# ParthaEth/GIF

Hardware: NVIDIA H100
Metric: G+D train step images/sec @256x256 bs32/GPU (higher is better)
Workload: dtype bf16x3 error-compensated tensor-core contraction (two-term bf16 operands, 3 MMAs per slice), f32 accumulate/storage

## Files before the change

### gif_b200/_lib.py

```python
import ctypes
import os

import torch

_HERE = os.path.dirname(os.path.abspath(__file__))
LIB_PATH = os.path.join(_HERE, "libgifb200.so")

_p = ctypes.c_void_p
_i = ctypes.c_int
_f = ctypes.c_float
_d = ctypes.c_double
_ll = ctypes.c_longlong
_sz = ctypes.c_size_t

SIGNATURES = {
    "gifb200_version": (_i, []),
    "gifb200_last_error": (ctypes.c_char_p, []),
    "gifb200_launch_count": (_ll, []),
    "gifb200_conv2d_workspace_bytes": (_sz, [_i] * 11),
    "gifb200_conv2d": (_i, [_p, _p, _p] + [_i] * 13 + [_p, _f, _f, _i, _p, _sz, _p]),
    "gifb200_conv2d_wgrad_workspace_bytes": (_sz, [_i] * 10),
    "gifb200_conv2d_wgrad_path": (_i, [_i] * 10),
    "gifb200_conv2d_wgrad": (_i, [_p, _p, _p] + [_i] * 12 + [_p, _sz, _p]),
    "gifb200_conv2d_ex_workspace_bytes": (_sz, [_i] * 13),
    "gifb200_conv2d_ex": (_i, [_p, _p, _p] + [_i] * 16 + [_p, _i, _p, _sz, _p]),
    "gifb200_pool2d": (_i, [_p, _p] + [_i] * 12 + [_p]),
    "gifb200_resize_bilinear": (_i, [_p, _p, _i, _i, _i, _ll, _ll, _ll, _ll, _i, _i, _i, _f, _f, _i, _p]),
    "gifb200_resize_bilinear_u8": (_i, [_p, _p, _i, _i, _i, _ll, _i, _i, _i, _f, _f, _i, _p]),
    "gifb200_split_bf16": (_i, [_p, _p, _p, _i, _i, _i, _p]),
    "gifb200_upfirdn2d": (_i, [_p, _p, _p] + [_i] * 14 + [_p]),
    "gifb200_bias_act": (_i, [_p, _p, _p, _p, _p, _i, _i, _i, _f, _f, _i, _p]),
    "gifb200_act_bwd": (_i, [_p, _p, _p, _ll, _f, _f, _i, _p]),
    "gifb200_rows_sum": (_i, [_p, _p, _i, _i, _i, _p]),
    "gifb200_chan_scale": (_i, [_p, _p, _p, _i, _i, _i, _i, _p]),
    "gifb200_tail_bwd": (_i, [_p] * 8 + [_i, _i, _i, _f, _f, _i, _p]),
    "gifb200_tail_bwd_planes": (_i, [_p] * 8 + [_i, _i, _i, _f, _f, _p, _p, _p]),
    "gifb200_scale_bwd": (_i, [_p] * 5 + [_i, _i, _i, _i, _p]),
    "gifb200_tail_bwd2": (_i, [_p] * 9 + [_i, _i, _i, _f, _f, _p, _p]),
    "gifb200_adam_step": (_i, [_p, _p, _p, _p, _p, _p, _i, _d, _d, _d, _d, _p]),
    "gifb200_spatial_dot": (_i, [_p, _p, _p, _i, _i, _i, _p]),
    "gifb200_axpby": (_i, [_p, _p, _p, _ll, _f, _f, _i, _p]),
    "gifb200_demod": (_i, [_p, _p, _p, _i, _i, _i, _f, _p]),
    "gifb200_torgb_fwd": (_i, [_p, _p, _p, _i, _i, _i, _p]),
    "gifb200_torgb_bwd_x": (_i, [_p, _p, _p, _i, _i, _i, _p]),
    "gifb200_torgb_bwd_w": (_i, [_p, _p, _p, _i, _i, _i, _p]),
    "gifb200_sgemm": (_i, [_i, _i, _i, _i, _i, _f, _p, _i, _p, _i, _p, _i, _p]),
    "gifb200_cond_down": (_i, [_p, _p, _i, _i, _i, _i, _i, _i, _p]),
    "gifb200_cond_up": (_i, [_p, _p, _i, _i, _i, _i, _i, _i, _p]),
    "gifb200_rasterize_workspace_bytes": (_sz, [_i, _i, _i, _i]),
    "gifb200_rasterize_fwd": (_i, [_p, _p, _p, _p, _p, _i, _i, _i, _i, _p, _sz, _p]),
    "gifb200_rasterize_fwd_ex": (_i, [_p] * 7 + [_i] * 5 + [_p, _sz, _p]),
    "gifb200_rasterize_bwd_ex": (_i, [_p] * 11 + [_i] * 5 + [_p]),
    "gifb200_render_shade": (_i, [_p] * 10 + [_i] * 5 + [_p]),
# ... 68 lines not shown
```

### gif_b200/csrc/conv_api.cu

```cuda
#include "common.cuh"

namespace gifb200 {
int conv2d_simt(const float* x, const float* w, float* y, int B, int Hi, int Wi, int Ci, int Ho, int Wo, int Co, int k,
                int mode, int flip, int transposed, const ConvEpilogue& epi, cudaStream_t st);
int conv2d_wgrad_simt(const float* x, const float* gy, float* gw, int B, int Hi, int Wi, int Ci, int Ho, int Wo, int Co,
                      int k, int mode, int flip, int transposed, cudaStream_t st);
bool conv2d_tc_supported(int B, int Hi, int Wi, int Ci, int Ho, int Wo, int Co, int k, int mode);
size_t conv2d_tc_workspace_bytes(int B, int Hi, int Wi, int Ci, int Ho, int Wo, int Co, int k, int mode, int transposed);
int conv2d_tc(const float* x, const float* w, float* y, int B, int Hi, int Wi, int Ci, int Ho, int Wo, int Co, int k,
              int mode, int flip, int transposed, const ConvEpilogue& epi, void* ws, size_t ws_bytes, cudaStream_t st,
              bool x3, bool prestaged);
bool conv2d_wgrad_tc_supported(int B, int Hi, int Wi, int Ci, int Ho, int Wo, int Co, int k, int mode);
size_t conv2d_wgrad_tc_workspace_bytes(int B, int Hi, int Wi, int Ci, int Ho, int Wo, int Co, int k, int mode);
int conv2d_wgrad_tc(const float* x, const float* gy, float* gw, int B, int Hi, int Wi, int Ci, int Ho, int Wo, int Co,
                    int k, int mode, int flip, int transposed, void* ws, size_t ws_bytes, cudaStream_t st, bool x3);
}

using namespace gifb200;

extern "C" size_t gifb200_conv2d_workspace_bytes(int B, int Hi, int Wi, int Ci, int Ho, int Wo, int Co, int k, int mode,
                                                 int transposed, int impl) {
    impl &= 0xF;
    if (impl == 1) return 0;
    if (!conv2d_tc_supported(B, Hi, Wi, Ci, Ho, Wo, Co, k, mode)) return 0;
    return conv2d_tc_workspace_bytes(B, Hi, Wi, Ci, Ho, Wo, Co, k, mode, transposed);
}

extern "C" int gifb200_conv2d(const float* x, const float* w, float* y, int B, int Hi, int Wi, int Ci, int Ho, int Wo,
                              int Co, int k, int mode, int flip, int transposed, int impl, int act, const float* bias,
                              float slope, float gain, int round_tf32, void* workspace, size_t workspace_bytes,
                              gifb200_stream_t stream) {
    cudaStream_t st = static_cast<cudaStream_t>(stream);
    const ConvEpilogue epi{act, bias, slope, gain, round_tf32};
    const bool prestaged = (impl & GIFB200_CONV_PRESTAGED) != 0;
    impl &= 0xF;
    GIFB200_REQUIRE(impl >= 0 && impl <= 3, GIFB200_E_SHAPE,
                    "conv2d: impl must be 0 (auto), 1 (simt), 2 (wgmma tf32) or 3 (wgmma bf16x3 on split planes)");
    const bool tc_ok = conv2d_tc_supported(B, Hi, Wi, Ci, Ho, Wo, Co, k, mode);
    if (impl >= 2 && !tc_ok) return fail(GIFB200_E_SHAPE, "conv2d: shape not supported by the tensor-core path");
    if (impl != 1 && tc_ok)
        return conv2d_tc(x, w, y, B, Hi, Wi, Ci, Ho, Wo, Co, k, mode, flip, transposed, epi, workspace, workspace_bytes, st,
                         impl == 3, prestaged);
    return conv2d_simt(x, w, y, B, Hi, Wi, Ci, Ho, Wo, Co, k, mode, flip, transposed, epi, st);
}

extern "C" size_t gifb200_conv2d_wgrad_workspace_bytes(int B, int Hi, int Wi, int Ci, int Ho, int Wo, int Co, int k,
                                                       int mode, int impl) {
    if (impl == 1) return 0;
    return conv2d_wgrad_tc_workspace_bytes(B, Hi, Wi, Ci, Ho, Wo, Co, k, mode);
}

extern "C" int gifb200_conv2d_wgrad_path(int B, int Hi, int Wi, int Ci, int Ho, int Wo, int Co, int k, int mode, int impl) {
    if (impl == 1) return 1;
    if (conv2d_wgrad_tc_supported(B, Hi, Wi, Ci, Ho, Wo, Co, k, mode)) return impl == 3 ? 3 : 2;
    return impl == 0 ? 1 : 0;
}

extern "C" int gifb200_conv2d_wgrad(const float* x, const float* gy, float* gw, int B, int Hi, int Wi, int Ci, int Ho,
                                    int Wo, int Co, int k, int mode, int flip, int transposed, int impl, void* workspace,
                                    size_t workspace_bytes, gifb200_stream_t stream) {
    GIFB200_REQUIRE(impl >= 0 && impl <= 3, GIFB200_E_SHAPE, "conv2d_wgrad: impl must be 0, 1, 2 or 3");
    const bool tc_ok = conv2d_wgrad_tc_supported(B, Hi, Wi, Ci, Ho, Wo, Co, k, mode);
    if (impl >= 2 && !tc_ok) return fail(GIFB200_E_SHAPE, "conv2d_wgrad: shape not supported by the tensor-core path");
    if (impl != 1 && tc_ok)
        return conv2d_wgrad_tc(x, gy, gw, B, Hi, Wi, Ci, Ho, Wo, Co, k, mode, flip, transposed, workspace,
                               workspace_bytes, static_cast<cudaStream_t>(stream), impl == 3);
    return conv2d_wgrad_simt(x, gy, gw, B, Hi, Wi, Ci, Ho, Wo, Co, k, mode, flip, transposed,
                             static_cast<cudaStream_t>(stream));
}
```

### gif_b200/csrc/conv_tc.cu

```cuda
#include <cuda_bf16.h>

#include "tc_common.cuh"

namespace gifb200 {

namespace {

constexpr int kBlockK = 32;
constexpr int kMaxTaps = 9;
constexpr int kConsumerWarps = 8;

struct TcParams {
    int B, Hs, Ws;
    int wt, ht, nt;
    int tiles_x, tiles_y;
    int Ci, Co;
    int s2;
    int Ho, Wo;
    int oys, oxs;
    int nphase;
    int phase_oy0[4], phase_ox0[4], phase_ntaps[4];
    int tap_w[4][kMaxTaps];
    int tap_dy[4][kMaxTaps];
    int tap_dx[4][kMaxTaps];
// ... 17 lines not shown
    static constexpr int kATileBytes = BM * kBlockK * 4;
    static constexpr int kBTileBytes = BN * kBlockK * 4;
    static constexpr int kStageBytes = kATileBytes + kBTileBytes;
    static constexpr int kBarrierOffset = kStages * kStageBytes;
    static constexpr int kTotal = kBarrierOffset + 16 * kStages;
    static constexpr int kDynamic = kTotal + 1024;
    static_assert(kDynamic <= 227 * 1024, "shared memory ring too large");
};

__device__ __forceinline__ void decode_tile(int tile, int nblocks, int nphase, int rot_div, int& mt, int& nblk, int& phase) {
    const int inner = nblocks * nphase;
    mt = tile / inner;
    const int rem = tile - mt * inner;
    nblk = rem % nblocks;
    phase = nphase == 1 ? 0 : (rem / nblocks + mt / rot_div) % nphase;
}

template <int BM, int BN, bool X3>
__global__ void __launch_bounds__(TileCfg<BM, BN>::kThreads, TileCfg<BM, BN>::kMinBlocks)
    conv_tc_kernel(const __grid_constant__ CUtensorMap map_a, const __grid_constant__ CUtensorMap map_a2,
                   const __grid_constant__ CUtensorMap map_b, const __grid_constant__ CUtensorMap map_b2,
                   float* __restrict__ y, const TcParams p, const int mtiles, const int total_tiles) {
    using L = TileCfg<BM, BN>;
    constexpr int kStages = L::kStages;
    constexpr int kATileBytes = L::kATileBytes;
    extern __shared__ uint8_t smem_raw[];
    uint8_t* smem = reinterpret_cast<uint8_t*>((reinterpret_cast<uintptr_t>(smem_raw) + 1023) & ~static_cast<uintptr_t>(1023));
    uint64_t* full_bar = reinterpret_cast<uint64_t*>(smem + L::kBarrierOffset);
    uint64_t* empty_bar = full_bar + kStages;

    const int warp = threadIdx.x >> 5, lane = threadIdx.x & 31;
    const int nblocks = p.Co / BN;
    const int kchunks = p.Ci / kBlockK;
    const int rot_div = max(1, static_cast<int>(gridDim.x) / (nblocks * p.nphase));
    (void)mtiles;

    if (warp == kConsumerWarps && lane == 0) {
        asm volatile("prefetch.tensormap [%0];" ::"l"(&map_a) : "memory");
        asm volatile("prefetch.tensormap [%0];" ::"l"(&map_b) : "memory");
        if (X3) {
            asm volatile("prefetch.tensormap [%0];" ::"l"(&map_a2) : "memory");
            asm volatile("prefetch.tensormap [%0];" ::"l"(&map_b2) : "memory");
        }
        for (int s = 0; s < kStages; ++s) { mbar_init(&full_bar[s], 1); mbar_init(&empty_bar[s], 2); }
        asm volatile("fence.mbarrier_init.release.cluster;" ::: "memory");
        asm volatile("fence.proxy.async.shared::cta;" ::: "memory");
    }
    __syncthreads();

    if (warp >= kConsumerWarps) {
        if constexpr (L::kLarge) setmaxnreg_dec<kProducerRegs>();
        if (warp != kConsumerWarps) return;
        int stage = 0;
        uint32_t ph = 0;
        for (int tile = blockIdx.x; tile < total_tiles; tile += gridDim.x) {
            int mt, nblk, phase;
            const int ks = tile % p.ksplit;
            decode_tile(tile / p.ksplit, nblocks, p.nphase, rot_div, mt, nblk, phase);
            int m = mt;
            const int tx = m % p.tiles_x; m /= p.tiles_x;
            const int ty = m % p.tiles_y; m /= p.tiles_y;
            const int n0 = m * p.nt, y0 = ty * p.ht, x0 = tx * p.wt;
            const int iters = p.phase_ntaps[phase] * kchunks;
            const int it0 = iters * ks / p.ksplit, it1 = iters * (ks + 1) / p.ksplit;
            for (int it = it0; it < it1; ++it) {
                const int tap = it / kchunks, c0 = (it % kchunks) * kBlockK;
                uint8_t* a_dst = smem + stage * L::kStageBytes;
                uint8_t* b_dst = a_dst + kATileBytes;
                if (lane == 0) {
                    mbar_wait(&empty_bar[stage], ph ^ 1);
                    mbar_expect_tx(&full_bar[stage], L::kStageBytes);
                }
                __syncwarp();
                const int dy = p.tap_dy[phase][tap], dx = p.tap_dx[phase][tap];
                if (!p.s2) {
                    if (lane == 0) {
                        tma_load_4d(a_dst, &map_a, &full_bar[stage], c0, x0 + dx, y0 + dy, n0);
                        if (X3) tma_load_4d(a_dst + kATileBytes / 2, &map_a2, &full_bar[stage], c0, x0 + dx, y0 + dy, n0);
                    }
                } else if (p.s2 == 2) {
                    if (lane == 0) {
                        const int par = p.tap_par[phase][tap];
                        tma_load_5d(a_dst, &map_a, &full_bar[stage], c0, par, x0 + dx, y0 * p.in_sy + dy, n0);
                        if (X3) tma_load_5d(a_dst + kATileBytes / 2, &map_a2, &full_bar[stage], c0, par, x0 + dx, y0 * p.in_sy + dy, n0);
                    }
                } else {
                    const int par = p.tap_par[phase][tap];
                    const int row_bytes = p.wt * kBlockK * (X3 ? 2 : 4);
                    const int rows = p.nt * p.ht;
                    for (int r = lane; r < rows; r += 32) {
                        const int n = r / p.ht, h = r - n * p.ht;
                        tma_load_5d(a_dst + r * row_bytes, &map_a, &full_bar[stage], c0, par, x0 + dx,
                                    (y0 + h) * p.in_sy + dy, n0 + n);
                        if (X3)
                            tma_load_5d(a_dst + kATileBytes / 2 + r * row_bytes, &map_a2, &full_bar[stage], c0, par, x0 + dx,
                                        (y0 + h) * p.in_sy + dy, n0 + n);
                    }
                }
                if (lane == 0) {
                    tma_load_3d(b_dst, &map_b, &full_bar[stage], c0, nblk * BN, p.tap_w[phase][tap]);
                    if (X3) tma_load_3d(b_dst + L::kBTileBytes / 2, &map_b2, &full_bar[stage], c0, nblk * BN, p.tap_w[phase][tap]);
                }
                if (++stage == kStages) { stage = 0; ph ^= 1; }
            }
        }
    } else {
        if constexpr (L::kLarge) setmaxnreg_inc<kConsumerRegs>();
        const int wg = warp >> 2;
        const int wq = warp & 3;
        constexpr int kRB = L::kRowBlocks;
        constexpr int kAcc = L::kAcc;
        float acc[kAcc];
        int w_in[2 * kRB], h_in[2 * kRB], n_in[2 * kRB];
#pragma unroll
        for (int rh = 0; rh < 2 * kRB; ++rh) {
            const int r = wg * (BM / 2) + (rh >> 1) * 64 + wq * 16 + (lane >> 2) + 8 * (rh & 1);
            w_in[rh] = r % p.wt; h_in[rh] = (r / p.wt) % p.ht; n_in[rh] = r / (p.wt * p.ht);
        }
        int stage = 0;
        uint32_t ph = 0;
        for (int tile = blockIdx.x; tile < total_tiles; tile += gridDim.x) {
            int mt, nblk, phase;
            const int ks = tile % p.ksplit;
            decode_tile(tile / p.ksplit, nblocks, p.nphase, rot_div, mt, nblk, phase);
            const int iters = p.phase_ntaps[phase] * kchunks;
            const int it0 = iters * ks / p.ksplit, it1 = iters * (ks + 1) / p.ksplit;
            int prev = -1;
            for (int it = it0; it < it1; ++it) {
                mbar_wait(&full_bar[stage], ph);
                const uint32_t a_addr = smem_u32(smem + stage * L::kStageBytes);
                wgmma_fence();
                fence_regs<kAcc>(acc);
                if (X3) {
                    const uint32_t a_wg = a_addr + wg * (BM / 2) * 64;
                    const uint64_t bh = make_kmajor_sw64_desc(a_addr + kATileBytes);
                    const uint64_t bl = make_kmajor_sw64_desc(a_addr + kATileBytes + L::kBTileBytes / 2);
#pragma unroll
                    for (int k = 0; k < kBlockK / 16; ++k) {
#pragma unroll
                        for (int rb = 0; rb < kRB; ++rb) {
                            const uint64_t ah = make_kmajor_sw64_desc(a_wg + rb * 64 * 64);
                            const uint64_t al = make_kmajor_sw64_desc(a_wg + rb * 64 * 64 + kATileBytes / 2);
                            float* d = acc + rb * (BN / 2);
                            wgmma_bf16<BN>(d, al + 2 * k, bh + 2 * k, (it != it0) || k != 0, Trans<0>());
                            wgmma_bf16<BN>(d, ah + 2 * k, bl + 2 * k, 1, Trans<0>());
                            wgmma_bf16<BN>(d, ah + 2 * k, bh + 2 * k, 1, Trans<0>());
                        }
                    }
                } else {
                    const uint64_t bdesc = make_kmajor_sw128_desc(a_addr + kATileBytes);
#pragma unroll
                    for (int k = 0; k < kBlockK / 8; ++k) {
#pragma unroll
                        for (int rb = 0; rb < kRB; ++rb) {
                            const uint64_t adesc = make_kmajor_sw128_desc(a_addr + (wg * (BM / 2) + rb * 64) * 128);
                            wgmma_tf32<BN>(acc + rb * (BN / 2), adesc + 2 * k, bdesc + 2 * k, (it != it0) || k != 0);
                        }
                    }
                }
                wgmma_commit();
                fence_regs<kAcc>(acc);
                wgmma_wait<1>();
                if (prev >= 0 && (threadIdx.x & 127) == 0) mbar_arrive(&empty_bar[prev]);
                prev = stage;
                if (++stage == kStages) { stage = 0; ph ^= 1; }
            }
            wgmma_wait<0>();
            fence_regs<kAcc>(acc);
            if (prev >= 0 && (threadIdx.x & 127) == 0) mbar_arrive(&empty_bar[prev]);
            int m = mt;
            const int tx = m % p.tiles_x; m /= p.tiles_x;
            const int ty = m % p.tiles_y; m /= p.tiles_y;
            float* base = p.ksplit > 1 ? p.part + ks * p.part_stride : y;
            const int c0 = nblk * BN + 2 * (lane & 3);
#pragma unroll
            for (int rh = 0; rh < 2 * kRB; ++rh) {
                const int h = rh & 1;
                const float* a = acc + (rh >> 1) * (BN / 2);
                const int n = m * p.nt + n_in[rh];
                const int Y = (ty * p.ht + h_in[rh]) * p.oys + p.phase_oy0[phase], X = (tx * p.wt + w_in[rh]) * p.oxs + p.phase_ox0[phase];
                if (n < p.B && Y < p.Ho && X < p.Wo) {
                    float* dst = base + ((static_cast<long long>(n) * p.Ho + Y) * p.Wo + X) * p.Co + c0;
#pragma unroll
                    for (int j = 0; j < BN / 8; ++j) {
                        float2 v = make_float2(a[4 * j + 2 * h], a[4 * j + 2 * h + 1]);
                        if (p.epi.act && p.ksplit == 1) {
                            v.x = apply_epilogue(p.epi, v.x, c0 + 8 * j);
                            v.y = apply_epilogue(p.epi, v.y, c0 + 8 * j + 1);
                        }
                        *reinterpret_cast<float2*>(dst + 8 * j) = v;
                    }
                }
            }
        }
    }
}

template <bool X3>
__global__ void __launch_bounds__(256) stage_weights_kernel(const float* __restrict__ w, float* __restrict__ out, int T,
                                                            int Co, int Ci, int flip, int transposed) {
    const long long total = static_cast<long long>(T) * Co * Ci;
    for (long long e = static_cast<long long>(blockIdx.x) * blockDim.x + threadIdx.x; e < total;
         e += static_cast<long long>(gridDim.x) * blockDim.x) {
        const int i = static_cast<int>(e % Ci);
        const int o = static_cast<int>((e / Ci) % Co);
        const int t = static_cast<int>(e / (static_cast<long long>(Ci) * Co));
        const int tt = flip ? T - 1 - t : t;
        const float v = transposed ? w[(static_cast<long long>(tt) * Ci + i) * Co + o]
                                   : w[(static_cast<long long>(tt) * Co + o) * Ci + i];
        if (X3) {
            __nv_bfloat16* planes = reinterpret_cast<__nv_bfloat16*>(out);
            const __nv_bfloat16 h = __float2bfloat16_rn(v);
            planes[e] = h;
            planes[total + e] = __float2bfloat16_rn(v - __bfloat162float(h));
        } else {
            out[e] = round_tf32(v);
        }
    }
}

__global__ void __launch_bounds__(256) splitk_reduce_kernel(const float* __restrict__ part, float* __restrict__ y, long long n4,
                                                            int ksplit, long long stride, ConvEpilogue epi, int Co) {
    for (long long i = static_cast<long long>(blockIdx.x) * blockDim.x + threadIdx.x; i < n4;
         i += static_cast<long long>(gridDim.x) * blockDim.x) {
        float4 a = __ldcs(reinterpret_cast<const float4*>(part) + i);
        for (int s = 1; s < ksplit; ++s) {
            const float4 b = __ldcs(reinterpret_cast<const float4*>(part + s * stride) + i);
// ... 45 lines not shown
    bn = lbn;
}

template <bool X3>
__global__ void __launch_bounds__(256) t2_corner_kernel(const void* __restrict__ xpix_v, const void* __restrict__ w22_v,
                                                        float* __restrict__ y, int B, long long x_batch_stride, int Ci, int Co,
                                                        int Ho, int Wo, ConvEpilogue epi, long long x_plane, long long w_plane) {
    const long long warp = (static_cast<long long>(blockIdx.x) * blockDim.x + threadIdx.x) >> 5;
    const int lane = threadIdx.x & 31;
    if (warp >= static_cast<long long>(B) * Co) return;
    const int b = static_cast<int>(warp / Co), o = static_cast<int>(warp % Co);
    float a = 0.f;
    if (X3) {
        const __nv_bfloat16* xv = static_cast<const __nv_bfloat16*>(xpix_v) + b * x_batch_stride;
        const __nv_bfloat16* wv = static_cast<const __nv_bfloat16*>(w22_v) + static_cast<long long>(o) * Ci;
        for (int i = lane; i < Ci; i += 32)
            a = fmaf(__bfloat162float(xv[i]) + __bfloat162float(xv[x_plane + i]),
                     __bfloat162float(wv[i]) + __bfloat162float(wv[w_plane + i]), a);
    } else {
        const float* xv = static_cast<const float*>(xpix_v) + b * x_batch_stride;
        const float* wv = static_cast<const float*>(w22_v) + static_cast<long long>(o) * Ci;
        for (int i = lane; i < Ci; i += 32) a = fmaf(xv[i], wv[i], a);
    }
    a = warp_sum(a);
    if (lane == 0) y[((static_cast<long long>(b) * Ho + (Ho - 1)) * Wo + (Wo - 1)) * Co + o] = apply_epilogue(epi, a, o);
}

void site_grid(int Hi, int Wi, int Ho, int Wo, int mode, int& Hs, int& Ws) {
    if (mode == 2) { Hs = Hi; Ws = Wi; } else { Hs = Ho; Ws = Wo; }
}

template <int BM, int BN, bool X3>
int launch(const CUtensorMap& ma, const CUtensorMap& ma2, const CUtensorMap& mb, const CUtensorMap& mb2, float* y,
           const TcParams& p, int mtiles, cudaStream_t st) {
    using L = TileCfg<BM, BN>;
    static bool attr_set = false;
    if (!attr_set) {
        cudaError_t e = cudaFuncSetAttribute(conv_tc_kernel<BM, BN, X3>, cudaFuncAttributeMaxDynamicSharedMemorySize, L::kDynamic);
        if (e != cudaSuccess) return fail(GIFB200_E_CUDA, "cudaFuncSetAttribute(conv_tc_kernel)", cudaGetErrorString(e));
        attr_set = true;
    }
    const long long total = static_cast<long long>(mtiles) * (p.Co / BN) * p.nphase * p.ksplit;
    if (total > 2147483647LL) return fail(GIFB200_E_SHAPE, "conv2d_tc: too many tiles");
    constexpr int kMaxGrid = L::kMinBlocks * kNumSMs;
    const int grid = total < kMaxGrid ? static_cast<int>(total) : kMaxGrid;
    conv_tc_kernel<BM, BN, X3><<<grid, L::kThreads, L::kDynamic, st>>>(ma, ma2, mb, mb2, y, p, mtiles, static_cast<int>(total));
    GIFB200_LAUNCH_CHECK("conv_tc_kernel");
    return GIFB200_OK;
}

template <bool X3>
int launch_tile(int bm, int bn, const CUtensorMap& ma, const CUtensorMap& ma2, const CUtensorMap& mb, const CUtensorMap& mb2,
                float* y, const TcParams& p, int mtiles, cudaStream_t st) {
    if (bm == 256) return launch<256, 128, X3>(ma, ma2, mb, mb2, y, p, mtiles, st);
    if (bn == 256) return launch<128, 256, X3>(ma, ma2, mb, mb2, y, p, mtiles, st);
    if (bn == 128) return launch<128, 128, X3>(ma, ma2, mb, mb2, y, p, mtiles, st);
    if (bn == 64) return launch<128, 64, X3>(ma, ma2, mb, mb2, y, p, mtiles, st);
    return launch<128, 32, X3>(ma, ma2, mb, mb2, y, p, mtiles, st);
}

int launch_any(int bm, int bn, bool x3, const CUtensorMap& ma, const CUtensorMap& ma2, const CUtensorMap& mb,
               const CUtensorMap& mb2, float* y, const TcParams& p, int mtiles, cudaStream_t st) {
    return x3 ? launch_tile<true>(bm, bn, ma, ma2, mb, mb2, y, p, mtiles, st)
              : launch_tile<false>(bm, bn, ma, ma2, mb, mb2, y, p, mtiles, st);
}

}

bool conv2d_tc_supported(int B, int Hi, int Wi, int Ci, int Ho, int Wo, int Co, int k, int mode) {
    if (B <= 0 || Ci % 32 != 0 || pick_block_n(Co) == 0) return false;
    if (!(k == 3 || (k == 1 && mode == 0))) return false;
    if (mode == 0 && !(Ho == Hi && Wo == Wi)) return false;
    if (mode == 1 && !(Hi == 2 * Ho + 1 && Wi == 2 * Wo + 1)) return false;
    if (mode == 2 && !(Ho == 2 * Hi + 1 && Wo == 2 * Wi + 1)) return false;
    int Hs, Ws;
    site_grid(Hi, Wi, Ho, Wo, mode, Hs, Ws);
    if (!pow2(Hs) || !pow2(Ws) || Ws < 4 || Hs < 4 || Ws > 4096 || Hs > 4096) return false;
    return true;
}

static size_t staged_weight_bytes(int Ci, int Co, int k) {
    return (static_cast<size_t>(k) * k * Co * Ci * sizeof(float) + 256 + 255) / 256 * 256;
}

static int ksplit_of(int B, int Hi, int Wi, int Ci, int Ho, int Wo, int Co, int k, int mode) {
    int Hs, Ws, wt, ht, nt;
    long long mtiles;
    site_grid(Hi, Wi, Ho, Wo, mode, Hs, Ws);
    tile_geometry(B, Hs, Ws, 128, wt, ht, nt, mtiles);
    const int bn = pick_block_n(Co);
    if (bn == 0) return 1;
    return pick_ksplit(mtiles * (Co / bn), k * k * (Ci / kBlockK), mode);
}

size_t conv2d_tc_workspace_bytes(int B, int Hi, int Wi, int Ci, int Ho, int Wo, int Co, int k, int mode, int) {
    size_t bytes = staged_weight_bytes(Ci, Co, k);
    if (conv2d_tc_supported(B, Hi, Wi, Ci, Ho, Wo, Co, k, mode)) {
        const int ks = ksplit_of(B, Hi, Wi, Ci, Ho, Wo, Co, k, mode);
        if (ks > 1) bytes += static_cast<size_t>(ks) * B * Ho * Wo * Co * sizeof(float) + 256;
    }
    return bytes;
}

int conv2d_tc(const float* x, const float* w, float* y, int B, int Hi, int Wi, int Ci, int Ho, int Wo, int Co, int k,
              int mode, int flip, int transposed, const ConvEpilogue& epi, void* ws, size_t ws_bytes, cudaStream_t st,
              bool x3, bool prestaged) {
    GIFB200_REQUIRE(conv2d_tc_supported(B, Hi, Wi, Ci, Ho, Wo, Co, k, mode), GIFB200_E_SHAPE, "conv2d_tc: unsupported shape");
    GIFB200_REQUIRE(ws && ws_bytes >= conv2d_tc_workspace_bytes(B, Hi, Wi, Ci, Ho, Wo, Co, k, mode, transposed),
                    GIFB200_E_WORKSPACE, "conv2d_tc: workspace too small (see gifb200_conv2d_workspace_bytes)");
    GIFB200_REQUIRE(aligned16(x) && aligned16(y), GIFB200_E_ALIGN, "conv2d_tc: x / y must be 16-byte aligned");
    const int T = k * k;
    float* wst = reinterpret_cast<float*>((reinterpret_cast<uintptr_t>(ws) + 255) & ~static_cast<uintptr_t>(255));
    if (!prestaged) {
        const long long total = static_cast<long long>(T) * Co * Ci;
        int blocks = cdiv(total, 256 * 4);
        if (blocks > kNumSMs * 4) blocks = kNumSMs * 4;
        if (x3) stage_weights_kernel<true><<<blocks, 256, 0, st>>>(w, wst, T, Co, Ci, flip, transposed);
        else stage_weights_kernel<false><<<blocks, 256, 0, st>>>(w, wst, T, Co, Ci, flip, transposed);
        GIFB200_LAUNCH_CHECK("stage_weights_kernel");
    }
    const cuuint64_t es = x3 ? 2 : 4;
    const CUtensorMapSwizzle swz = x3 ? CU_TENSOR_MAP_SWIZZLE_64B : CU_TENSOR_MAP_SWIZZLE_128B;
    const CUtensorMapDataType dt = x3 ? CU_TENSOR_MAP_DATA_TYPE_BFLOAT16 : CU_TENSOR_MAP_DATA_TYPE_FLOAT32;
    const long long x_plane = static_cast<long long>(B) * Hi * Wi * Ci;
    const long long w_plane = static_cast<long long>(T) * Co * Ci;
// ... 46 lines not shown
    if (mode != 1) {
        const cuuint64_t dims[4] = {static_cast<cuuint64_t>(Ci), static_cast<cuuint64_t>(Wi), static_cast<cuuint64_t>(Hi), static_cast<cuuint64_t>(B)};
        const cuuint64_t strides[3] = {static_cast<cuuint64_t>(Ci) * es, static_cast<cuuint64_t>(Wi) * Ci * es,
                                       static_cast<cuuint64_t>(Hi) * Wi * Ci * es};
        const cuuint32_t box[4] = {kBlockK, static_cast<cuuint32_t>(p.wt), static_cast<cuuint32_t>(p.ht), static_cast<cuuint32_t>(p.nt)};
        rc = encode_map(&ma, xb, 4, dims, strides, box, swz, dt);
        if (rc == GIFB200_OK && x3) rc = encode_map(&ma2, xb + x_plane * es, 4, dims, strides, box, swz, dt);
    } else {
        const cuuint64_t dims[5] = {static_cast<cuuint64_t>(Ci), 2, static_cast<cuuint64_t>((Wi + 1) / 2), static_cast<cuuint64_t>(Hi), static_cast<cuuint64_t>(B)};
        const cuuint64_t strides[4] = {static_cast<cuuint64_t>(Ci) * es, static_cast<cuuint64_t>(Ci) * 2 * es,
                                       static_cast<cuuint64_t>(Wi) * Ci * es, static_cast<cuuint64_t>(Hi) * Wi * Ci * es};
        static const bool per_row = [] { const char* e = getenv("GIFB200_CONV_S2_ROWS"); return e && atoi(e) != 0; }();
        const bool onebox = !per_row && p.ht * p.nt > 1;
        if (onebox) p.s2 = 2;
        const cuuint32_t box[5] = {kBlockK, 1, static_cast<cuuint32_t>(p.wt), static_cast<cuuint32_t>(onebox ? 2 * p.ht : 1),
                                   static_cast<cuuint32_t>(onebox ? p.nt : 1)};
        const cuuint32_t estr[5] = {1, 1, 1, static_cast<cuuint32_t>(onebox ? 2 : 1), 1};
        rc = encode_map(&ma, xb, 5, dims, strides, box, swz, dt, estr);
        if (rc == GIFB200_OK && x3) rc = encode_map(&ma2, xb + x_plane * es, 5, dims, strides, box, swz, dt, estr);
    }
    if (rc != GIFB200_OK) return rc;
    auto encode_b = [&](int box_n, CUtensorMap& m, CUtensorMap& m2) {
        const cuuint64_t dims[3] = {static_cast<cuuint64_t>(Ci), static_cast<cuuint64_t>(Co), static_cast<cuuint64_t>(T)};
        const cuuint64_t strides[2] = {static_cast<cuuint64_t>(Ci) * es, static_cast<cuuint64_t>(Co) * Ci * es};
        const cuuint32_t box[3] = {kBlockK, static_cast<cuuint32_t>(box_n), 1};
        int r = encode_map(&m, wb, 3, dims, strides, box, swz, dt);
        if (r == GIFB200_OK && x3) r = encode_map(&m2, wb + w_plane * es, 3, dims, strides, box, swz, dt);
        if (!x3) m2 = m;
        return r;
    };
    rc = encode_b(bn, mb, mb2);
    if (rc != GIFB200_OK) return rc;
    if (!x3) ma2 = ma;
    rc = launch_any(bm, bn, x3, ma, ma2, mb, mb2, y, p, static_cast<int>(mtiles), st);
    if (rc == GIFB200_OK && p.ksplit > 1) {
        const long long n4 = p.part_stride / 4;
        int blocks = cdiv(n4, 256);
        if (blocks > kNumSMs * 8) blocks = kNumSMs * 8;
        splitk_reduce_kernel<<<blocks, 256, 0, st>>>(p.part, y, n4, p.ksplit, p.part_stride, epi, Co);
        GIFB200_LAUNCH_CHECK("splitk_reduce_kernel");
    }
    if (mode != 2 || rc != GIFB200_OK) return rc;
    const int bn_e = pick_block_n(Co);
    CUtensorMap mbe = mb, mbe2 = mb2;
    if (bn_e != bn) rc = encode_b(bn_e, mbe, mbe2);
    for (int edge = 0; edge < 2 && rc == GIFB200_OK; ++edge) {
        const bool row = edge == 0;
        TcParams q;
        memset(&q, 0, sizeof(q));
        q.B = B; q.Ci = Ci; q.Co = Co; q.Ho = Ho; q.Wo = Wo; q.epi = epi;
        q.Hs = row ? 1 : Hi; q.Ws = row ? Wi : 1;
        q.wt = q.Ws < 128 ? q.Ws : 128;
        q.ht = (128 / q.wt) < q.Hs ? (128 / q.wt) : q.Hs;
        q.nt = 128 / (q.wt * q.ht);
        q.tiles_x = q.Ws / q.wt; q.tiles_y = q.Hs / q.ht;
        const long long mt_e = static_cast<long long>(q.tiles_x) * q.tiles_y * ((B + q.nt - 1) / q.nt);
        q.s2 = 0; q.in_sy = 1; q.nphase = 2; q.oys = q.oxs = 2; q.ksplit = 1;
        for (int ph = 0; ph < 2; ++ph) {
            q.phase_oy0[ph] = row ? 2 * Hi : ph;
            q.phase_ox0[ph] = row ? ph : 2 * Wi;
            int n = 0;
            for (int kk = ph; kk < 3; kk += 2) {
                q.tap_w[ph][n] = row ? (2 * 3 + kk) : (kk * 3 + 2);
                q.tap_dy[ph][n] = row ? 0 : (ph - kk) / 2;
                q.tap_dx[ph][n] = row ? (ph - kk) / 2 : 0;
                ++n;
            }
            q.phase_ntaps[ph] = n;
        }
        CUtensorMap me, me2;
        const char* base = xb + (row ? static_cast<long long>(Hi - 1) * Wi * Ci : static_cast<long long>(Wi - 1) * Ci) * es;
        const cuuint64_t dims[4] = {static_cast<cuuint64_t>(Ci), static_cast<cuuint64_t>(row ? Wi : 1),
                                    static_cast<cuuint64_t>(row ? 1 : Hi), static_cast<cuuint64_t>(B)};
        const cuuint64_t strides[3] = {static_cast<cuuint64_t>(Ci) * es, static_cast<cuuint64_t>(Wi) * Ci * es,
                                       static_cast<cuuint64_t>(Hi) * Wi * Ci * es};
        const cuuint32_t box[4] = {kBlockK, static_cast<cuuint32_t>(q.wt), static_cast<cuuint32_t>(q.ht), static_cast<cuuint32_t>(q.nt)};
        rc = encode_map(&me, base, 4, dims, strides, box, swz, dt);
        if (rc == GIFB200_OK && x3) rc = encode_map(&me2, base + x_plane * es, 4, dims, strides, box, swz, dt);
        if (rc != GIFB200_OK) return rc;
        if (!x3) me2 = me;
        rc = launch_any(128, bn_e, x3, me, me2, mbe, mbe2, y, q, static_cast<int>(mt_e), st);
    }
    if (rc != GIFB200_OK) return rc;
    {
        const char* xpix = xb + (static_cast<long long>(Hi - 1) * Wi + (Wi - 1)) * Ci * es;
        const char* w22 = wb + static_cast<long long>(8) * Co * Ci * es;
        const int blocks = cdiv(static_cast<long long>(B) * Co * 32, 256);
        if (x3)
            t2_corner_kernel<true><<<blocks, 256, 0, st>>>(xpix, w22, y, B, static_cast<long long>(Hi) * Wi * Ci, Ci, Co, Ho, Wo,
                                                           epi, x_plane, w_plane);
        else
            t2_corner_kernel<false><<<blocks, 256, 0, st>>>(xpix, w22, y, B, static_cast<long long>(Hi) * Wi * Ci, Ci, Co, Ho, Wo,
                                                            epi, 0, 0);
    }
    GIFB200_LAUNCH_CHECK("t2_corner_kernel");
    return rc;
}

}
```

### gif_b200/csrc/tc_common.cuh

```cuda
#pragma once
#include <cuda.h>

#include <mutex>

#include "common.cuh"

namespace gifb200 {

__device__ __forceinline__ uint32_t smem_u32(const void* p) { return static_cast<uint32_t>(__cvta_generic_to_shared(p)); }

__device__ __forceinline__ void mbar_init(uint64_t* bar, uint32_t count) {
    asm volatile("mbarrier.init.shared::cta.b64 [%0], %1;" ::"r"(smem_u32(bar)), "r"(count));
}
__device__ __forceinline__ void mbar_expect_tx(uint64_t* bar, uint32_t bytes) {
    asm volatile("mbarrier.arrive.expect_tx.shared::cta.b64 _, [%0], %1;" ::"r"(smem_u32(bar)), "r"(bytes) : "memory");
}
__device__ __forceinline__ void mbar_arrive(uint64_t* bar) {
    asm volatile("mbarrier.arrive.shared::cta.b64 _, [%0];" ::"r"(smem_u32(bar)) : "memory");
}

__device__ __forceinline__ void mbar_wait(uint64_t* bar, uint32_t parity) {
    asm volatile(
        "{\n"
        ".reg .pred p;\n"
        "WAIT_LOOP:\n"
        "mbarrier.try_wait.parity.shared::cta.b64 p, [%0], %1;\n"
        "@p bra WAIT_DONE;\n"
        "bra WAIT_LOOP;\n"
        "WAIT_DONE:\n"
        "}\n" ::"r"(smem_u32(bar)),
        "r"(parity)
        : "memory");
}
__device__ __forceinline__ void tma_load_3d(void* dst, const CUtensorMap* map, uint64_t* bar, int c0, int c1, int c2) {
    asm volatile(
        "cp.async.bulk.tensor.3d.shared::cluster.global.mbarrier::complete_tx::bytes [%0], [%1, {%3, %4, %5}], [%2];"
        ::"r"(smem_u32(dst)), "l"(map), "r"(smem_u32(bar)), "r"(c0), "r"(c1), "r"(c2)
        : "memory");
}
__device__ __forceinline__ void tma_load_4d(void* dst, const CUtensorMap* map, uint64_t* bar, int c0, int c1, int c2,
                                            int c3) {
    asm volatile(
        "cp.async.bulk.tensor.4d.shared::cluster.global.mbarrier::complete_tx::bytes [%0], [%1, {%3, %4, %5, %6}], [%2];"
        ::"r"(smem_u32(dst)), "l"(map), "r"(smem_u32(bar)), "r"(c0), "r"(c1), "r"(c2), "r"(c3)
        : "memory");
}
__device__ __forceinline__ void tma_load_5d(void* dst, const CUtensorMap* map, uint64_t* bar, int c0, int c1, int c2,
                                            int c3, int c4) {
    asm volatile(
        "cp.async.bulk.tensor.5d.shared::cluster.global.mbarrier::complete_tx::bytes [%0], [%1, {%3, %4, %5, %6, %7}], [%2];"
        ::"r"(smem_u32(dst)), "l"(map), "r"(smem_u32(bar)), "r"(c0), "r"(c1), "r"(c2), "r"(c3), "r"(c4)
        : "memory");
}
__device__ __forceinline__ void wgmma_fence() { asm volatile("wgmma.fence.sync.aligned;" ::: "memory"); }
__device__ __forceinline__ void wgmma_commit() { asm volatile("wgmma.commit_group.sync.aligned;" ::: "memory"); }
template <int N>
__device__ __forceinline__ void wgmma_wait() { asm volatile("wgmma.wait_group.sync.aligned %0;" ::"n"(N) : "memory"); }
template <int R>
__device__ __forceinline__ void setmaxnreg_inc() { asm volatile("setmaxnreg.inc.sync.aligned.u32 %0;" ::"n"(R)); }
template <int R>
__device__ __forceinline__ void setmaxnreg_dec() { asm volatile("setmaxnreg.dec.sync.aligned.u32 %0;" ::"n"(R)); }
template <int R>
__device__ __forceinline__ void fence_regs(float* d) {
#pragma unroll
    for (int i = 0; i < R; ++i) asm volatile("" : "+f"(d[i])::"memory");
}
template <int V>
struct Trans {};
template <int N>
__device__ __forceinline__ void wgmma_tf32(float* d, uint64_t da, uint64_t db, int scale_d);
template <int N, int T>
__device__ __forceinline__ void wgmma_bf16(float* d, uint64_t da, uint64_t db, int scale_d, Trans<T>);
#define GIF_F8(i) "+f"(d[i]), "+f"(d[i + 1]), "+f"(d[i + 2]), "+f"(d[i + 3]), "+f"(d[i + 4]), "+f"(d[i + 5]), "+f"(d[i + 6]), "+f"(d[i + 7])
#define GIF_F16 GIF_F8(0), GIF_F8(8)
#define GIF_F32 GIF_F16, GIF_F8(16), GIF_F8(24)
#define GIF_F64 GIF_F32, GIF_F8(32), GIF_F8(40), GIF_F8(48), GIF_F8(56)
#define GIF_R8(a, b, c, d, e, f, g, h) "%" #a ", %" #b ", %" #c ", %" #d ", %" #e ", %" #f ", %" #g ", %" #h
#define GIF_R16 GIF_R8(0, 1, 2, 3, 4, 5, 6, 7) ", " GIF_R8(8, 9, 10, 11, 12, 13, 14, 15)
#define GIF_R32 GIF_R16 ", " GIF_R8(16, 17, 18, 19, 20, 21, 22, 23) ", " GIF_R8(24, 25, 26, 27, 28, 29, 30, 31)
#define GIF_R64 GIF_R32 ", " GIF_R8(32, 33, 34, 35, 36, 37, 38, 39) ", " GIF_R8(40, 41, 42, 43, 44, 45, 46, 47) ", " \
    GIF_R8(48, 49, 50, 51, 52, 53, 54, 55) ", " GIF_R8(56, 57, 58, 59, 60, 61, 62, 63)
#define GIF_F128 GIF_F64, GIF_F8(64), GIF_F8(72), GIF_F8(80), GIF_F8(88), GIF_F8(96), GIF_F8(104), GIF_F8(112), GIF_F8(120)
#define GIF_R128 GIF_R64 ", " GIF_R8(64, 65, 66, 67, 68, 69, 70, 71) ", " GIF_R8(72, 73, 74, 75, 76, 77, 78, 79) ", " \
    GIF_R8(80, 81, 82, 83, 84, 85, 86, 87) ", " GIF_R8(88, 89, 90, 91, 92, 93, 94, 95) ", " \
    GIF_R8(96, 97, 98, 99, 100, 101, 102, 103) ", " GIF_R8(104, 105, 106, 107, 108, 109, 110, 111) ", " \
    GIF_R8(112, 113, 114, 115, 116, 117, 118, 119) ", " GIF_R8(120, 121, 122, 123, 124, 125, 126, 127)
// ... 106 lines not shown
```

### include/gifb200.h

```cpp
#ifndef GIFB200_H
#define GIFB200_H

#include <stddef.h>
#include <stdint.h>

#ifdef __cplusplus
extern "C" {
#endif

#define GIFB200_OK 0
#define GIFB200_E_SHAPE (-1)
#define GIFB200_E_ALIGN (-2)
#define GIFB200_E_ARCH (-3)
#define GIFB200_E_CUDA (-4)
#define GIFB200_E_WORKSPACE (-5)

typedef void* gifb200_stream_t;

int gifb200_version(void);
const char* gifb200_last_error(void);
long long gifb200_launch_count(void);

#define GIFB200_CONV_PRESTAGED 0x10
size_t gifb200_conv2d_workspace_bytes(int B, int Hi, int Wi, int Ci, int Ho, int Wo, int Co, int k, int mode,
                                      int transposed, int impl);
int gifb200_conv2d(const float* x, const float* w, float* y, int B, int Hi, int Wi, int Ci, int Ho, int Wo, int Co,
                   int k, int mode, int flip, int transposed, int impl, int act, const float* bias, float slope,
                   float gain, int round_tf32, void* workspace, size_t workspace_bytes, gifb200_stream_t stream);

size_t gifb200_conv2d_wgrad_workspace_bytes(int B, int Hi, int Wi, int Ci, int Ho, int Wo, int Co, int k, int mode,
                                            int impl);
int gifb200_conv2d_wgrad_path(int B, int Hi, int Wi, int Ci, int Ho, int Wo, int Co, int k, int mode, int impl);
int gifb200_conv2d_wgrad(const float* x, const float* gy, float* gw, int B, int Hi, int Wi, int Ci, int Ho, int Wo,
                         int Co, int k, int mode, int flip, int transposed, int impl, void* workspace,
                         size_t workspace_bytes, gifb200_stream_t stream);

size_t gifb200_conv2d_ex_workspace_bytes(int B, int Hi, int Wi, int Ci, int Ho, int Wo, int Co, int kh, int kw, int stride,
                                         int pad_h, int pad_w, int impl);
int gifb200_conv2d_ex(const void* x, const float* w, float* y, int B, int Hi, int Wi, int Ci, int Ho, int Wo, int Co, int kh,
                      int kw, int stride, int pad_h, int pad_w, int Cy, int c0, int impl, int act, const float* bias,
                      int round_tf32, void* workspace, size_t workspace_bytes, gifb200_stream_t stream);
int gifb200_pool2d(const float* x, float* y, int B, int Hi, int Wi, int C, int Ho, int Wo, int stride, int pad, int op, int Cy,
                   int c0, int round_tf32, gifb200_stream_t stream);
int gifb200_resize_bilinear(const float* x, float* y, int B, int H, int W, long long stride_b, long long stride_c,
                            long long stride_h, long long stride_w, int Ho, int Wo, int Cy, float scale, float shift,
                            int round_tf32, gifb200_stream_t stream);
int gifb200_resize_bilinear_u8(const uint8_t* x, float* y, int B, int H, int W, long long stride_b, int Ho, int Wo, int Cy,
                               float scale, float shift, int round_tf32, gifb200_stream_t stream);

int gifb200_split_bf16(const float* x, const float* s, void* planes, int B, int P, int C, gifb200_stream_t stream);

int gifb200_upfirdn2d(const float* x, const float* kernel, float* y, int B, int Hi, int Wi, int C, int Ho, int Wo,
                      int kh, int kw, int up, int down, int pad_y0, int pad_x0, int flip, int round_tf32,
                      gifb200_stream_t stream);

int gifb200_bias_act(const float* x, const float* rowscale, const float* add, const float* bias, float* y, int B,
                     int P, int C, float slope, float gain, int round_tf32, gifb200_stream_t stream);
int gifb200_act_bwd(const float* gy, const float* y, float* gx, long long n, float slope, float gain,
                    int round_tf32, gifb200_stream_t stream);
int gifb200_rows_sum(const float* x, float* out, int G, int rows, int C, gifb200_stream_t stream);
int gifb200_chan_scale(const float* x, const float* s, float* y, int B, int P, int C, int round_tf32,
// ... 98 lines not shown
```

Measured before the change: 82.00.

## Pair large conv tiles into 2-CTA clusters with multicast weight TMA loads

Large tensor-core conv tiles now launch as 2-CTA thread block clusters that share the same weight block. Each CTA TMA-loads half of the B tile and multicasts it to both CTAs, with cross-CTA empty-barrier arrivals and a drain at exit. The aim is to halve global/L2 traffic for weight operands per M-tile pair. In exchange it adds cluster synchronisation and scheduling constraints, and an odd tile count may leave a CTA doing unused work.

```diff
diff --git a/gif_b200/_lib.py b/gif_b200/_lib.py
--- a/gif_b200/_lib.py
+++ b/gif_b200/_lib.py
@@ -19,6 +19,7 @@
     "gifb200_launch_count": (_ll, []),
     "gifb200_conv2d_workspace_bytes": (_sz, [_i] * 11),
     "gifb200_conv2d": (_i, [_p, _p, _p] + [_i] * 13 + [_p, _f, _f, _i, _p, _sz, _p]),
+    "gifb200_conv2d_cluster_size": (_i, [_i] * 10),
     "gifb200_conv2d_wgrad_workspace_bytes": (_sz, [_i] * 10),
     "gifb200_conv2d_wgrad_path": (_i, [_i] * 10),
     "gifb200_conv2d_wgrad": (_i, [_p, _p, _p] + [_i] * 12 + [_p, _sz, _p]),
diff --git a/gif_b200/csrc/conv_api.cu b/gif_b200/csrc/conv_api.cu
--- a/gif_b200/csrc/conv_api.cu
+++ b/gif_b200/csrc/conv_api.cu
@@ -7,6 +7,7 @@
                       int k, int mode, int flip, int transposed, cudaStream_t st);
 bool conv2d_tc_supported(int B, int Hi, int Wi, int Ci, int Ho, int Wo, int Co, int k, int mode);
 size_t conv2d_tc_workspace_bytes(int B, int Hi, int Wi, int Ci, int Ho, int Wo, int Co, int k, int mode, int transposed);
+int conv2d_tc_cluster_size(int B, int Hi, int Wi, int Ci, int Ho, int Wo, int Co, int k, int mode);
 int conv2d_tc(const float* x, const float* w, float* y, int B, int Hi, int Wi, int Ci, int Ho, int Wo, int Co, int k,
               int mode, int flip, int transposed, const ConvEpilogue& epi, void* ws, size_t ws_bytes, cudaStream_t st,
               bool x3, bool prestaged);
@@ -44,6 +45,12 @@
     return conv2d_simt(x, w, y, B, Hi, Wi, Ci, Ho, Wo, Co, k, mode, flip, transposed, epi, st);
 }
 
+extern "C" int gifb200_conv2d_cluster_size(int B, int Hi, int Wi, int Ci, int Ho, int Wo, int Co, int k, int mode, int impl) {
+    impl &= 0xF;
+    if (impl == 1 || impl > 3 || !conv2d_tc_supported(B, Hi, Wi, Ci, Ho, Wo, Co, k, mode)) return 0;
+    return conv2d_tc_cluster_size(B, Hi, Wi, Ci, Ho, Wo, Co, k, mode);
+}
+
 extern "C" size_t gifb200_conv2d_wgrad_workspace_bytes(int B, int Hi, int Wi, int Ci, int Ho, int Wo, int Co, int k,
                                                        int mode, int impl) {
     if (impl == 1) return 0;
diff --git a/gif_b200/csrc/conv_tc.cu b/gif_b200/csrc/conv_tc.cu
--- a/gif_b200/csrc/conv_tc.cu
+++ b/gif_b200/csrc/conv_tc.cu
@@ -73,7 +73,11 @@
     const int warp = threadIdx.x >> 5, lane = threadIdx.x & 31;
     const int nblocks = p.Co / BN;
     const int kchunks = p.Ci / kBlockK;
-    const int rot_div = max(1, static_cast<int>(gridDim.x) / (nblocks * p.nphase));
+    auto csize = [] { return L::kLarge ? static_cast<int>(cluster_nctarank()) : 1; };
+    auto crank = [] { return L::kLarge ? static_cast<int>(cluster_ctarank()) : 0; };
+    auto cid = [] { return L::kLarge ? static_cast<int>(cluster_id_x()) : static_cast<int>(blockIdx.x); };
+    auto ccount = [] { return L::kLarge ? static_cast<int>(cluster_count_x()) : static_cast<int>(gridDim.x); };
+    const int rot_div = max(1, ccount() / (nblocks * p.nphase));
     (void)mtiles;
 
     if (warp == kConsumerWarps && lane == 0) {
@@ -83,21 +87,23 @@
             asm volatile("prefetch.tensormap [%0];" ::"l"(&map_a2) : "memory");
             asm volatile("prefetch.tensormap [%0];" ::"l"(&map_b2) : "memory");
         }
-        for (int s = 0; s < kStages; ++s) { mbar_init(&full_bar[s], 1); mbar_init(&empty_bar[s], 2); }
+        for (int s = 0; s < kStages; ++s) { mbar_init(&full_bar[s], 1); mbar_init(&empty_bar[s], 2 * csize()); }
         asm volatile("fence.mbarrier_init.release.cluster;" ::: "memory");
         asm volatile("fence.proxy.async.shared::cta;" ::: "memory");
     }
     __syncthreads();
+    if (csize() > 1) cluster_sync();
 
     if (warp >= kConsumerWarps) {
         if constexpr (L::kLarge) setmaxnreg_dec<kProducerRegs>();
         if (warp != kConsumerWarps) return;
         int stage = 0;
         uint32_t ph = 0;
-        for (int tile = blockIdx.x; tile < total_tiles; tile += gridDim.x) {
+        for (int tile = cid(); tile < total_tiles; tile += ccount()) {
             int mt, nblk, phase;
             const int ks = tile % p.ksplit;
             decode_tile(tile / p.ksplit, nblocks, p.nphase, rot_div, mt, nblk, phase);
+            mt = mt * csize() + crank();
             int m = mt;
             const int tx = m % p.tiles_x; m /= p.tiles_x;
             const int ty = m % p.tiles_y; m /= p.tiles_y;
@@ -139,8 +145,16 @@
                     }
                 }
                 if (lane == 0) {
-                    tma_load_3d(b_dst, &map_b, &full_bar[stage], c0, nblk * BN, p.tap_w[phase][tap]);
-                    if (X3) tma_load_3d(b_dst + L::kBTileBytes / 2, &map_b2, &full_bar[stage], c0, nblk * BN, p.tap_w[phase][tap]);
+                    const int tw = p.tap_w[phase][tap];
+                    if (csize() == 1) {
+                        tma_load_3d(b_dst, &map_b, &full_bar[stage], c0, nblk * BN, tw);
+                        if (X3) tma_load_3d(b_dst + L::kBTileBytes / 2, &map_b2, &full_bar[stage], c0, nblk * BN, tw);
+                    } else {
+                        const int off = crank() * (L::kBTileBytes / (X3 ? 4 : 2));
+                        const int row = nblk * BN + crank() * (BN / 2);
+                        tma_load_3d_multicast(b_dst + off, &map_b, &full_bar[stage], c0, row, tw, 0x3);
+                        if (X3) tma_load_3d_multicast(b_dst + L::kBTileBytes / 2 + off, &map_b2, &full_bar[stage], c0, row, tw, 0x3);
+                    }
                 }
                 if (++stage == kStages) { stage = 0; ph ^= 1; }
             }
@@ -158,12 +172,17 @@
             const int r = wg * (BM / 2) + (rh >> 1) * 64 + wq * 16 + (lane >> 2) + 8 * (rh & 1);
             w_in[rh] = r % p.wt; h_in[rh] = (r / p.wt) % p.ht; n_in[rh] = r / (p.wt * p.ht);
         }
+        auto release = [&](int s) {
+            mbar_arrive(&empty_bar[s]);
+            if (csize() > 1) mbar_arrive_cluster(&empty_bar[s], crank() ^ 1);
+        };
         int stage = 0;
         uint32_t ph = 0;
-        for (int tile = blockIdx.x; tile < total_tiles; tile += gridDim.x) {
+        for (int tile = cid(); tile < total_tiles; tile += ccount()) {
             int mt, nblk, phase;
             const int ks = tile % p.ksplit;
             decode_tile(tile / p.ksplit, nblocks, p.nphase, rot_div, mt, nblk, phase);
+            mt = mt * csize() + crank();
             const int iters = p.phase_ntaps[phase] * kchunks;
             const int it0 = iters * ks / p.ksplit, it1 = iters * (ks + 1) / p.ksplit;
             int prev = -1;
@@ -202,13 +221,13 @@
                 wgmma_commit();
                 fence_regs<kAcc>(acc);
                 wgmma_wait<1>();
-                if (prev >= 0 && (threadIdx.x & 127) == 0) mbar_arrive(&empty_bar[prev]);
+                if (prev >= 0 && (threadIdx.x & 127) == 0) release(prev);
                 prev = stage;
                 if (++stage == kStages) { stage = 0; ph ^= 1; }
             }
             wgmma_wait<0>();
             fence_regs<kAcc>(acc);
-            if (prev >= 0 && (threadIdx.x & 127) == 0) mbar_arrive(&empty_bar[prev]);
+            if (prev >= 0 && (threadIdx.x & 127) == 0) release(prev);
             int m = mt;
             const int tx = m % p.tiles_x; m /= p.tiles_x;
             const int ty = m % p.tiles_y; m /= p.tiles_y;
@@ -234,6 +253,12 @@
                 }
             }
         }
+        if (csize() > 1 && threadIdx.x == 0) {
+            for (int s = 0; s < kStages; ++s) {
+                mbar_wait(&empty_bar[stage], ph ^ 1);
+                if (++stage == kStages) { stage = 0; ph ^= 1; }
+            }
+        }
     }
 }
 
@@ -345,37 +370,69 @@
 
 template <int BM, int BN, bool X3>
 int launch(const CUtensorMap& ma, const CUtensorMap& ma2, const CUtensorMap& mb, const CUtensorMap& mb2, float* y,
-           const TcParams& p, int mtiles, cudaStream_t st) {
+           const TcParams& p, int mtiles, int cs, cudaStream_t st) {
     using L = TileCfg<BM, BN>;
     static bool attr_set = false;
+    static int max_pairs = 0;
     if (!attr_set) {
         cudaError_t e = cudaFuncSetAttribute(conv_tc_kernel<BM, BN, X3>, cudaFuncAttributeMaxDynamicSharedMemorySize, L::kDynamic);
         if (e != cudaSuccess) return fail(GIFB200_E_CUDA, "cudaFuncSetAttribute(conv_tc_kernel)", cudaGetErrorString(e));
         attr_set = true;
     }
-    const long long total = static_cast<long long>(mtiles) * (p.Co / BN) * p.nphase * p.ksplit;
+    const long long units = cs == 2 ? (mtiles + 1) / 2 : mtiles;
+    const long long total = units * (p.Co / BN) * p.nphase * p.ksplit;
     if (total > 2147483647LL) return fail(GIFB200_E_SHAPE, "conv2d_tc: too many tiles");
-    constexpr int kMaxGrid = L::kMinBlocks * kNumSMs;
-    const int grid = total < kMaxGrid ? static_cast<int>(total) : kMaxGrid;
-    conv_tc_kernel<BM, BN, X3><<<grid, L::kThreads, L::kDynamic, st>>>(ma, ma2, mb, mb2, y, p, mtiles, static_cast<int>(total));
+    if (cs == 1) {
+        constexpr int kMaxGrid = L::kMinBlocks * kNumSMs;
+        const int grid = total < kMaxGrid ? static_cast<int>(total) : kMaxGrid;
+        conv_tc_kernel<BM, BN, X3><<<grid, L::kThreads, L::kDynamic, st>>>(ma, ma2, mb, mb2, y, p, mtiles, static_cast<int>(total));
+        GIFB200_LAUNCH_CHECK("conv_tc_kernel");
+        return GIFB200_OK;
+    }
+    if (!L::kLarge || p.ksplit != 1) return fail(GIFB200_E_SHAPE, "conv2d_tc: CTA pairs need a large tile without split-K");
+    cudaLaunchConfig_t cfg = {};
+    cudaLaunchAttribute attr[1];
+    attr[0].id = cudaLaunchAttributeClusterDimension;
+    attr[0].val.clusterDim.x = 2;
+    attr[0].val.clusterDim.y = 1;
+    attr[0].val.clusterDim.z = 1;
+    cfg.blockDim = dim3(L::kThreads);
+    cfg.dynamicSmemBytes = L::kDynamic;
+    cfg.stream = st;
+    cfg.attrs = attr;
+    cfg.numAttrs = 1;
+    if (max_pairs == 0) {
+        cfg.gridDim = dim3(2 * kNumSMs);
+        cudaError_t e = cudaOccupancyMaxActiveClusters(&max_pairs, conv_tc_kernel<BM, BN, X3>, &cfg);
+        if (e != cudaSuccess) return fail(GIFB200_E_CUDA, "cudaOccupancyMaxActiveClusters(conv_tc_kernel)", cudaGetErrorString(e));
+        if (max_pairs < 1) return fail(GIFB200_E_CUDA, "conv_tc_kernel: no cluster of two CTAs fits on the device");
+    }
+    cfg.gridDim = dim3(static_cast<unsigned>(2 * (total < max_pairs ? total : max_pairs)));
+    cudaError_t e = cudaLaunchKernelEx(&cfg, conv_tc_kernel<BM, BN, X3>, ma, ma2, mb, mb2, y, p, mtiles, static_cast<int>(total));
+    if (e != cudaSuccess) return fail(GIFB200_E_CUDA, "cudaLaunchKernelEx(conv_tc_kernel)", cudaGetErrorString(e));
     GIFB200_LAUNCH_CHECK("conv_tc_kernel");
     return GIFB200_OK;
 }
 
 template <bool X3>
 int launch_tile(int bm, int bn, const CUtensorMap& ma, const CUtensorMap& ma2, const CUtensorMap& mb, const CUtensorMap& mb2,
-                float* y, const TcParams& p, int mtiles, cudaStream_t st) {
-    if (bm == 256) return launch<256, 128, X3>(ma, ma2, mb, mb2, y, p, mtiles, st);
-    if (bn == 256) return launch<128, 256, X3>(ma, ma2, mb, mb2, y, p, mtiles, st);
-    if (bn == 128) return launch<128, 128, X3>(ma, ma2, mb, mb2, y, p, mtiles, st);
-    if (bn == 64) return launch<128, 64, X3>(ma, ma2, mb, mb2, y, p, mtiles, st);
-    return launch<128, 32, X3>(ma, ma2, mb, mb2, y, p, mtiles, st);
+                float* y, const TcParams& p, int mtiles, int cs, cudaStream_t st) {
+    if (bm == 256) return launch<256, 128, X3>(ma, ma2, mb, mb2, y, p, mtiles, cs, st);
+    if (bn == 256) return launch<128, 256, X3>(ma, ma2, mb, mb2, y, p, mtiles, cs, st);
+    if (bn == 128) return launch<128, 128, X3>(ma, ma2, mb, mb2, y, p, mtiles, cs, st);
+    if (bn == 64) return launch<128, 64, X3>(ma, ma2, mb, mb2, y, p, mtiles, cs, st);
+    return launch<128, 32, X3>(ma, ma2, mb, mb2, y, p, mtiles, cs, st);
 }
 
 int launch_any(int bm, int bn, bool x3, const CUtensorMap& ma, const CUtensorMap& ma2, const CUtensorMap& mb,
-               const CUtensorMap& mb2, float* y, const TcParams& p, int mtiles, cudaStream_t st) {
-    return x3 ? launch_tile<true>(bm, bn, ma, ma2, mb, mb2, y, p, mtiles, st)
-              : launch_tile<false>(bm, bn, ma, ma2, mb, mb2, y, p, mtiles, st);
+               const CUtensorMap& mb2, float* y, const TcParams& p, int mtiles, int cs, cudaStream_t st) {
+    return x3 ? launch_tile<true>(bm, bn, ma, ma2, mb, mb2, y, p, mtiles, cs, st)
+              : launch_tile<false>(bm, bn, ma, ma2, mb, mb2, y, p, mtiles, cs, st);
+}
+
+int cluster_size(int bm, int bn) {
+    static const bool single = [] { const char* e = getenv("GIFB200_CONV_CLUSTER"); return e && atoi(e) == 1; }();
+    return bm * bn > 128 * 128 && !single ? 2 : 1;
 }
 
 }
@@ -404,6 +461,13 @@
     const int bn = pick_block_n(Co);
     if (bn == 0) return 1;
     return pick_ksplit(mtiles * (Co / bn), k * k * (Ci / kBlockK), mode);
+}
+
+int conv2d_tc_cluster_size(int B, int Hi, int Wi, int Ci, int Ho, int Wo, int Co, int k, int mode) {
+    int Hs, Ws, bm, bn;
+    site_grid(Hi, Wi, Ho, Wo, mode, Hs, Ws);
+    pick_tile(B, Hs, Ws, Co, mode == 2 ? 4 : 1, ksplit_of(B, Hi, Wi, Ci, Ho, Wo, Co, k, mode), bm, bn);
+    return cluster_size(bm, bn);
 }
 
 size_t conv2d_tc_workspace_bytes(int B, int Hi, int Wi, int Ci, int Ho, int Wo, int Co, int k, int mode, int) {
@@ -516,7 +580,14 @@
     rc = encode_b(bn, mb, mb2);
     if (rc != GIFB200_OK) return rc;
     if (!x3) ma2 = ma;
-    rc = launch_any(bm, bn, x3, ma, ma2, mb, mb2, y, p, static_cast<int>(mtiles), st);
+    const int cs = cluster_size(bm, bn);
+    if (cs == 1) {
+        rc = launch_any(bm, bn, x3, ma, ma2, mb, mb2, y, p, static_cast<int>(mtiles), 1, st);
+    } else {
+        CUtensorMap mbh, mbh2;
+        rc = encode_b(bn / 2, mbh, mbh2);
+        if (rc == GIFB200_OK) rc = launch_any(bm, bn, x3, ma, ma2, mbh, mbh2, y, p, static_cast<int>(mtiles), cs, st);
+    }
     if (rc == GIFB200_OK && p.ksplit > 1) {
         const long long n4 = p.part_stride / 4;
         int blocks = cdiv(n4, 256);
@@ -563,7 +634,7 @@
         if (rc == GIFB200_OK && x3) rc = encode_map(&me2, base + x_plane * es, 4, dims, strides, box, swz, dt);
         if (rc != GIFB200_OK) return rc;
         if (!x3) me2 = me;
-        rc = launch_any(128, bn_e, x3, me, me2, mbe, mbe2, y, q, static_cast<int>(mt_e), st);
+        rc = launch_any(128, bn_e, x3, me, me2, mbe, mbe2, y, q, static_cast<int>(mt_e), 1, st);
     }
     if (rc != GIFB200_OK) return rc;
     {
diff --git a/gif_b200/csrc/tc_common.cuh b/gif_b200/csrc/tc_common.cuh
--- a/gif_b200/csrc/tc_common.cuh
+++ b/gif_b200/csrc/tc_common.cuh
@@ -52,6 +52,44 @@
         ::"r"(smem_u32(dst)), "l"(map), "r"(smem_u32(bar)), "r"(c0), "r"(c1), "r"(c2), "r"(c3), "r"(c4)
         : "memory");
 }
+__device__ __forceinline__ void tma_load_3d_multicast(void* dst, const CUtensorMap* map, uint64_t* bar, int c0, int c1, int c2,
+                                                      uint16_t cta_mask) {
+    asm volatile(
+        "cp.async.bulk.tensor.3d.shared::cluster.global.mbarrier::complete_tx::bytes.multicast::cluster"
+        " [%0], [%1, {%3, %4, %5}], [%2], %6;"
+        ::"r"(smem_u32(dst)), "l"(map), "r"(smem_u32(bar)), "r"(c0), "r"(c1), "r"(c2), "h"(cta_mask)
+        : "memory");
+}
+
+__device__ __forceinline__ uint32_t cluster_nctarank() {
+    uint32_t r;
+    asm volatile("mov.u32 %0, %%cluster_nctarank;" : "=r"(r));
+    return r;
+}
+__device__ __forceinline__ uint32_t cluster_ctarank() {
+    uint32_t r;
+    asm volatile("mov.u32 %0, %%cluster_ctarank;" : "=r"(r));
+    return r;
+}
+__device__ __forceinline__ uint32_t cluster_id_x() {
+    uint32_t r;
+    asm volatile("mov.u32 %0, %%clusterid.x;" : "=r"(r));
+    return r;
+}
+__device__ __forceinline__ uint32_t cluster_count_x() {
+    uint32_t r;
+    asm volatile("mov.u32 %0, %%nclusterid.x;" : "=r"(r));
+    return r;
+}
+__device__ __forceinline__ void cluster_sync() {
+    asm volatile("barrier.cluster.arrive.release;\nbarrier.cluster.wait.acquire;" ::: "memory");
+}
+__device__ __forceinline__ void mbar_arrive_cluster(uint64_t* bar, uint32_t rank) {
+    uint32_t remote;
+    asm volatile("mapa.shared::cluster.u32 %0, %1, %2;" : "=r"(remote) : "r"(smem_u32(bar)), "r"(rank));
+    asm volatile("mbarrier.arrive.shared::cluster.b64 _, [%0];" ::"r"(remote) : "memory");
+}
+
 __device__ __forceinline__ void wgmma_fence() { asm volatile("wgmma.fence.sync.aligned;" ::: "memory"); }
 __device__ __forceinline__ void wgmma_commit() { asm volatile("wgmma.commit_group.sync.aligned;" ::: "memory"); }
 template <int N>
diff --git a/include/gifb200.h b/include/gifb200.h
--- a/include/gifb200.h
+++ b/include/gifb200.h
@@ -27,6 +27,7 @@
 int gifb200_conv2d(const float* x, const float* w, float* y, int B, int Hi, int Wi, int Ci, int Ho, int Wo, int Co,
                    int k, int mode, int flip, int transposed, int impl, int act, const float* bias, float slope,
                    float gain, int round_tf32, void* workspace, size_t workspace_bytes, gifb200_stream_t stream);
+int gifb200_conv2d_cluster_size(int B, int Hi, int Wi, int Ci, int Ho, int Wo, int Co, int k, int mode, int impl);
 
 size_t gifb200_conv2d_wgrad_workspace_bytes(int B, int Hi, int Wi, int Ci, int Ho, int Wo, int Co, int k, int mode,
                                             int impl);
```

Result: no change. 82.56, median of 6 (+0.7%).
